# cold-deuu/Quadrotor_Manipulator_MPPI

Measured on AMD Instinct MI355X. Metric: MPPI rollouts/sec (K x H state-steps) + control-step p50 latency, K=4096 H=32, higher is better.
Workload: dtype f32

## Files before the change

quadrotor_manipulator_mppi_amd/csrc/mppi_finalize.hip:

```cpp
#include <algorithm>

#include "mppi_device.h"

using namespace mppi;

constexpr int kFinThreads = 512;
constexpr int kMaxRec = 4096;
#ifndef MPPI_FIN_KO
#define MPPI_FIN_KO 0
#endif
#ifndef MPPI_FIN_NOMARK
#define MPPI_FIN_NOMARK 0
#endif
#ifndef MPPI_FIN_XCDS
#define MPPI_FIN_XCDS 8
#endif
#ifndef MPPI_FIN_QUIET_LEAN
#define MPPI_FIN_QUIET_LEAN 1
#endif

#if defined(MPPI_STAMPS) && !defined(MPPI_TIMELINE)
#define FSTAMP(i)                                                                    \
    do {                                                                             \
        __builtin_amdgcn_sched_barrier(0);                                           \
        if (pk.stamps && threadIdx.x == 0)                                           \
            pk.stamps[(((size_t)v * A + a) * ts + sl) * kStamps + (i)] =               \
                __builtin_amdgcn_s_memtime();                                        \
        __builtin_amdgcn_sched_barrier(0);                                           \
    } while (0)
#define FSTAMPRT(i) do { } while (0)
#elif defined(MPPI_STAMPS)
#define FSTAMPRT(i)                                                                  \
    do {                                                                             \
        if (pk.stamps && threadIdx.x == 0) {                                         \
            pk.stamps[(((size_t)v * A + a) * ts + sl) * kStamps + (i)] =               \
                __builtin_amdgcn_s_memrealtime();                                    \
            if ((i) == 13)                                                           \
                pk.stamps[(((size_t)v * A + a) * ts + sl) * kStamps + 15] =            \
                    (unsigned long long)__builtin_amdgcn_s_getreg(0xF814);           \
        }                                                                            \
    } while (0)
#define FSTAMP(i) do { if ((i) == 1 || (i) == 7) FSTAMPRT(i); } while (0)
#else
#define FSTAMP(i) do { } while (0)
#define FSTAMPRT(i) do { } while (0)
#endif

enum { kRoleAny = 0, kRoleFinal = 1, kRoleQuiet = 2, kRolePack = 3, kRolePeer = 4 };
struct GeoRt { static constexpr bool kStatic = false; static constexpr int A = 0, H = 0, tsz = 0, hf = 0, ts = 0; };
template <int A_, int H_, int TSZ_, int HF_, int TS_>
struct GeoC { static constexpr bool kStatic = true; static constexpr int A = A_, H = H_, tsz = TSZ_, hf = HF_, ts = TS_; };

template <int CW, int WIN, int NT, int ROLE, typename GEO, int CPL = 1>
__device__ __forceinline__ void fin_body(const float* __restrict__ hdr_base, const float* __restrict__ dat_base,
                                         const FinTail* __restrict__ tail, const uint32_t nrec_H, const uint32_t geo,
                                         const int32_t hdr_rs, const int32_t d_rs, const int32_t d_as,
                                         const int32_t hdr_vs, const int32_t d_vs, const uint32_t seq_arg,
                                         const FinParams& pk) {
    constexpr bool kAny = ROLE == kRoleAny, kQuiet = ROLE == kRoleQuiet;
    constexpr bool kOut = kAny || ROLE == kRoleFinal || ROLE == kRolePeer;
    constexpr bool kUpd = kOut || kQuiet;
    constexpr bool kPeer = kAny || ROLE == kRolePeer;
    constexpr bool kEta2 = !(kQuiet && MPPI_FIN_QUIET_LEAN);
    constexpr int NWV = NT / 64;
    constexpr int ROWS = 64 / CW;
    constexpr int TR = NWV * ROWS;
    constexpr int kNPT = 16;
    static_assert(CPL == 1 || ((CPL == 2 || CPL == 4) && CW == 16 && NT / CPL >= 32), "lane maps: see above");
    constexpr int LPR = CW / CPL;
    constexpr int kLanes = NT / CPL < 64 ? NT / CPL : 64;
    __shared__ float wcol[NWV][CW];
    __shared__ float wrho[NWV], wnan[NWV], weta[NWV], weta2[NWV];
    __shared__ float wsg[96];
    const FinParams& p = pk;
    const int tid = threadIdx.x, lane = tid & 63, wv = tid >> 6;
    const int n = (int)(nrec_H & 0xFFFFu);
    const int H = GEO::kStatic ? GEO::H : (int)(nrec_H >> 16);
    const int tsz = GEO::kStatic ? GEO::tsz : (int)(geo & 0xFFu), hf = GEO::kStatic ? GEO::hf : (int)((geo >> 8) & 0xFFu);
    const int ts = GEO::kStatic ? GEO::ts : (int)((geo >> 16) & 0xFFu), A = GEO::kStatic ? GEO::A : (int)(geo >> 24);
    const int x8 = blockIdx.x & 7, j8 = blockIdx.x >> 3, na = (A + MPPI_FIN_XCDS - 1) / MPPI_FIN_XCDS;
    const int sl = (na == 1) ? j8 : (na == 2) ? (j8 >> 1) : j8 / na;
    const int a = x8 + MPPI_FIN_XCDS * (j8 - sl * na), v = blockIdx.y;
    if (x8 >= MPPI_FIN_XCDS || a >= A) return;
    if (MPPI_FIN_KO & 16) { if (tid == 0) p.u_prev[blockIdx.x] = 0.0f; return; }
    FSTAMPRT(13);
    FSTAMP(0);
// ... 94 lines not shown
            }
            if (wv == 0 && xpeers)
                xpl = ((const __attribute__((address_space(1))) unsigned long long*)xpeers)[lane < xn ? lane : 0];
        }
    };
    float rho_t = INFINITY, nanflag = 0.0f, eta = 0.0f, eta2 = 0.0f;
    float acc[CPL];
#pragma unroll
    for (int j = 0; j < CPL; ++j) acc[j] = 0.0f;
    const uint32_t hrs_b = (uint32_t)hdr_rs * 4u, drs_b = (uint32_t)d_rs * 4u;
    const __amdgpu_buffer_rsrc_t hrsrc =
        __builtin_amdgcn_make_buffer_rsrc(const_cast<float*>(hdr), 0, __builtin_amdgcn_readfirstlane((int)((uint32_t)n * hrs_b)),
                                          0x00020000);
    const __amdgpu_buffer_rsrc_t crsrc = __builtin_amdgcn_make_buffer_rsrc(
        const_cast<float*>(col), 0,
        __builtin_amdgcn_readfirstlane((int)((uint32_t)(n - 1) * drs_b + (uint32_t)(CPL == 1 ? W : nqd * CPL) * 4u)),
        0x00020000);
    typedef uint32_t u32x4 __attribute__((ext_vector_type(4)));
    typedef uint32_t u32x2 __attribute__((ext_vector_type(2)));
    for (int base = 0; base < n; base += TR * kNPT) {
        float4 hd[kNPT];
        float xv[kNPT][CPL];
        uint32_t okm = 0;
        const uint32_t r0 = (uint32_t)(base + gr);
        const uint32_t hoff = r0 * hrs_b, coff = r0 * drs_b + (uint32_t)(qv ? q : 0) * (uint32_t)(4 * CPL);
#pragma unroll
        for (int i = 0; i < kNPT; ++i) {
            okm |= (uint32_t)(r0 + (uint32_t)(i * TR) < (uint32_t)n) << i;
            const u32x4 h = __builtin_amdgcn_raw_buffer_load_b128(hrsrc, (int)(hoff + (uint32_t)(i * TR) * hrs_b), 0, kAuxDev);
            hd[i] = make_float4(__uint_as_float(h.x), __uint_as_float(h.y), __uint_as_float(h.z), __uint_as_float(h.w));
            const int bo = (int)(coff + (uint32_t)(i * TR) * drs_b);
            if constexpr (CPL == 4) {
                const u32x4 b = __builtin_amdgcn_raw_buffer_load_b128(crsrc, bo, 0, kAuxDev);
                xv[i][0] = __uint_as_float(b.x); xv[i][1] = __uint_as_float(b.y);
                xv[i][2] = __uint_as_float(b.z); xv[i][3] = __uint_as_float(b.w);
            } else if constexpr (CPL == 2) {
                const u32x2 b = __builtin_amdgcn_raw_buffer_load_b64(crsrc, bo, 0, kAuxDev);
                xv[i][0] = __uint_as_float(b.x); xv[i][1] = __uint_as_float(b.y);
            } else {
                xv[i][0] = __uint_as_float(__builtin_amdgcn_raw_buffer_load_b32(crsrc, bo, 0, kAuxDev));
            }
        }
        if (base == 0) {
            __builtin_amdgcn_sched_barrier(0);
            pin_tail();
        }
#pragma unroll
        for (int i = 0; i < kNPT; ++i)
            if (!((okm >> i) & 1u)) hd[i].x = INFINITY;
        FSTAMP(7);
        float m = INFINITY;
#pragma unroll
        for (int i = 0; i < kNPT; ++i) { m = fminf(m, hd[i].x); nanflag = fmaxf(nanflag, hd[i].w); }
        if constexpr (!kEta2) {
#pragma unroll
            for (int i = 0; i < kNPT; ++i) asm volatile("" :: "v"(hd[i].z));
        }
        float fr[kNPT];
#pragma unroll
        for (int i = 0; i < kNPT; ++i) fr[i] = 0.0f;
        if (m < INFINITY) {
            const float rn = fminf(rho_t, m);
            if (rho_t < INFINITY) {
                const float sc = __expf(coef * (rho_t - rn));
#pragma unroll
                for (int j = 0; j < CPL; ++j) acc[j] *= sc;
                eta *= sc;
                if constexpr (kEta2) eta2 *= sc * sc;
            }
            rho_t = rn;
#pragma unroll
            for (int i = 0; i < kNPT; ++i) {
                const float f = (hd[i].x < INFINITY) ? __expf(coef * (hd[i].x - rn)) : 0.0f;
                fr[i] = f;
                eta = fmaf(f, hd[i].y, eta);
                if constexpr (kEta2) eta2 = fmaf(f * f, hd[i].z, eta2);
            }
        }
#pragma unroll
        for (int i = 0; i < kNPT; ++i) {
#pragma unroll
            for (int j = 0; j < CPL; ++j) acc[j] = fmaf(fr[i], xv[i][j], acc[j]);
        }
        FSTAMP(8);
    }
    if constexpr (CPL == 1) {
        const float rw = fold_rows<CW>(rho_t, OpMin());
        const float sc = (rho_t < INFINITY) ? __expf(coef * (rho_t - rw)) : 0.0f;
        acc[0] = fold_rows<CW>(acc[0] * sc, OpAdd());
        const float e1 = fold_rows<CW>(eta * sc, OpAdd()), e2 = fold_rows<CW>(eta2 * (sc * sc), OpAdd());
        const float nf = fold_rows<CW>(nanflag, OpMax());
        if (lane < CW) wcol[wv][lane] = acc[0];
        if (lane == 0) { wrho[wv] = rw; wnan[wv] = nf; weta[wv] = e1; weta2[wv] = e2; }
    } else {
        auto fold_g = [](float x, auto op) {
            asm volatile("" : "+v"(x));
// ... 434 lines not shown
```

quadrotor_manipulator_mppi_amd/csrc/mppi_host_math.cpp:

```cpp
#include <algorithm>
#include <cmath>
#include <cstdarg>
#include <cstdio>
#include <cstring>
#include <string>
#include <vector>

#include "mppi_engine.h"

using namespace mppi;

namespace {
thread_local std::string g_err;

template <typename T>
void base_from_xyzquat_t(const double* b, float* T16) {
    const T qx = (T)b[3], qy = (T)b[4], qz = (T)b[5], qw = (T)b[6];
    volatile T a, c;
    std::memset(T16, 0, 16 * sizeof(float));
    a = (T)1 - (T)2 * (qy * qy); a = a - (T)2 * (qz * qz); T16[0] = (float)a;
    a = ((T)2 * qx) * qy; c = ((T)2 * qz) * qw; T16[1] = (float)(a - c);
    a = ((T)2 * qx) * qz; c = ((T)2 * qy) * qw; T16[2] = (float)(a + c);
    a = ((T)2 * qx) * qy; c = ((T)2 * qz) * qw; T16[4] = (float)(a + c);
    a = (T)1 - (T)2 * (qx * qx); a = a - (T)2 * (qz * qz); T16[5] = (float)a;
// ... 219 lines not shown
        if (!(c.quad_mass > 0.0f) || !(c.quad_inertia[0] > 0.0f) || !(c.quad_inertia[1] > 0.0f) ||
            !(c.quad_inertia[2] > 0.0f))
            return fail(MPPI_ERR_INVALID_ARG, "QUADROTOR needs a positive mass and inertia");
    }
    if (c.model == MPPI_MODEL_ARM || c.model == MPPI_MODEL_WHOLEBODY) {
        if (c.n_joints < 1 || c.n_joints > MPPI_MAX_JOINTS)
            return fail(MPPI_ERR_INVALID_ARG, "n_joints=%d", c.n_joints);
        const int nq = nq_of(c);
        for (int j = 0; j < c.n_joints; ++j) {
            const mppi_joint& jj = c.joints[j];
            if (jj.type < 0 || jj.type > 2) return fail(MPPI_ERR_INVALID_ARG, "joint %d: bad type", j);
            if (jj.type != MPPI_JOINT_FIXED && (jj.q_index < 0 || jj.q_index >= nq))
                return fail(MPPI_ERR_INVALID_ARG, "joint %d: q_index %d outside [0,%d)", j, jj.q_index, nq);
        }
    }
    const int half = c.savgol_window / 2;
    if (c.savgol_window % 2 != 1 || c.savgol_window > kMaxW)
        return fail(MPPI_ERR_INVALID_ARG, "Window size must be odd (and <= %d).", kMaxW);
    if (c.savgol_order >= c.savgol_window)
        return fail(MPPI_ERR_INVALID_ARG, "Polyorder must be less than window size.");
    if (c.n_horizon <= half)
        return fail(MPPI_ERR_INVALID_ARG, "Padding (%d) is too large for data length (%d).", half, c.n_horizon);
    if (!(c.lambda_ > 0.0) || !(c.dt > 0.0)) return fail(MPPI_ERR_INVALID_ARG, "lambda and dt must be > 0");
    if (c.shard_count < 1 || c.shard_rank < 0 || c.shard_rank >= c.shard_count)
        return fail(MPPI_ERR_INVALID_ARG, "shard %d/%d", c.shard_rank, c.shard_count);
    if ((int64_t)c.shard_count * (int64_t)c.n_samples > (int64_t)1 << 32)
        return fail(MPPI_ERR_INVALID_ARG, "shard_count %d x n_samples %d = %lld samples: the 32-bit sample counter of "
                    "the noise stream addresses at most 2^32", c.shard_count, c.n_samples,
                    (long long)c.shard_count * (long long)c.n_samples);
    if (c.vehicle_offset < 0 || c.vehicle_offset + c.n_vehicles > 32768)
        return fail(MPPI_ERR_INVALID_ARG, "vehicle_offset %d: the fleet-wide vehicle index must stay below 32768",
                    c.vehicle_offset);
    if (c.cost_terms & ~0x3F) return fail(MPPI_ERR_INVALID_ARG, "unknown cost_terms bits 0x%x", c.cost_terms);
    if ((c.cost_terms & 0x1F) && (c.model == MPPI_MODEL_DRONE || c.model == MPPI_MODEL_QUADROTOR))
        return fail(MPPI_ERR_INVALID_ARG, "cost_terms apply to the ARM / WHOLEBODY CostManager (not DRONE)");
    if (c.block_threads && (c.block_threads % 64 || c.block_threads > 512))
        return fail(MPPI_ERR_INVALID_ARG, "block_threads must be a multiple of 64 <= 512");
    return MPPI_OK;
}

}

using namespace mppi_host;

extern "C" {

// ... 122 lines not shown
```

quadrotor_manipulator_mppi_amd/csrc/mppi_rollout.h:

```cpp
#pragma once
#include "mppi_device.h"

#ifndef MPPI_KO
#define MPPI_KO 0
#endif
#ifndef MPPI_ROLL_OCC_NCH2
#define MPPI_ROLL_OCC_NCH2 4
#endif
#ifndef MPPI_ROLL_OCC_NCH2_XC
#define MPPI_ROLL_OCC_NCH2_XC 2
#endif
#ifndef MPPI_ROLL_OCC_XC
#define MPPI_ROLL_OCC_XC 4
#endif
#ifndef MPPI_ROLL_OCC
#define MPPI_ROLL_OCC 4
#endif
#ifndef MPPI_PRIO
#define MPPI_PRIO 1
#endif
#ifndef MPPI_S_PLAIN
#define MPPI_S_PLAIN 0
#endif
#ifndef MPPI_EPS_STASH
#define MPPI_EPS_STASH 1
#endif
#ifndef MPPI_COMB_EXIT
#define MPPI_COMB_EXIT 0
#endif
#ifndef MPPI_QUIET_LEAN
#define MPPI_QUIET_LEAN 1
#endif
#ifndef MPPI_FK_PRETRIG
#define MPPI_FK_PRETRIG 1
#endif

namespace {

__device__ __forceinline__ uint32_t xor3_sk(uint32_t a, uint32_t b, uint32_t k) {
    uint32_t r;
    asm("v_bitop3_b32 %0, %1, %2, %3 bitop3:0x96" : "=v"(r) : "v"(a), "v"(b), "s"(k));
    return r;
}

__device__ __forceinline__ void philox10(uint32_t& c0, uint32_t& c1, uint32_t& c2, uint32_t& c3,
                                         uint32_t k0, uint32_t k1) {
    k0 = __builtin_amdgcn_readfirstlane(k0);
    k1 = __builtin_amdgcn_readfirstlane(k1);
#pragma unroll
    for (int r = 0; r < 10; ++r) {
        if (r) {
            asm volatile("s_add_u32 %0, %0, 0x9e3779b9" : "+s"(k0) :: "scc");
            asm volatile("s_add_u32 %0, %0, 0xbb67ae85" : "+s"(k1) :: "scc");
        }
        const uint64_t p0 = (uint64_t)0xD2511F53u * c0;
        const uint64_t p1 = (uint64_t)0xCD9E8D57u * c2;
        const uint32_t n0 = xor3_sk((uint32_t)(p1 >> 32), c1, k0), n2 = xor3_sk((uint32_t)(p0 >> 32), c3, k1);
        c0 = n0; c1 = (uint32_t)p1; c2 = n2; c3 = (uint32_t)p0;
    }
// ... 520 lines not shown
#pragma unroll
        for (int j = 0; j < NU; ++j)
            ur[j] = __uint_as_float(__builtin_amdgcn_raw_buffer_load_b32(urs, (tid + j * nthr) * 4, 0, kAuxDev));
    };
    if (!ovl) load_u();
    if (MODEL != MPPI_MODEL_DRONE) {
        const int* js = (const int*)jtab;
#pragma unroll
        for (int j = 0; j < NJ; ++j) {
            const int i = tid + j * nthr;
            jr[j] = (i < kJW) ? js[i] : 0;
        }
    }
    constexpr int kVCW = (int)(sizeof(VehicleConst) / 4);
    const int vcr = (tid < kVCW) ? (VONE ? ((const int*)&pk.vc0)[tid] : ((const int*)(pk.vc + v))[tid]) : 0;
    float tgt[TRK ? NCH : 1][12];
    if constexpr (TRK) {
#pragma unroll
        for (int c = 0; c < NCH; ++c) {
            const int t = t0 + 64 * c, tc = (t < H_arg) ? t : H_arg - 1;
            load_target_row<MODEL == MPPI_MODEL_DRONE>(ttab + ((size_t)v * H_arg + tc) * 12, tgt[c]);
        }
    }
    uint32_t kwarm = 0u;
    {
        const uint32_t* kp = (const uint32_t*)&pk;
#pragma unroll
        for (int o = 0; o < (int)(offsetof(DevParams, sigma) / 4); o += 16) kwarm ^= kp[o];
    }
    STAMPW(9);
    float z0[NCH][NA];
    SECTION("prologue_philox");
    if (noise_mode != MPPI_NOISE_INJECTED) {
        const uint32_t kg = k_off + (uint32_t)((blockIdx.x * nw + wid) * R + sub);
#pragma unroll
        for (int c = 0; c < NCH; ++c)
            draw_normals<NA>(z0[c], kg, (uint32_t)(t0 + 64 * c), vkey, step_ctr, seed_lo, seed_hi);
    }
    if (ovl) {
        if (wid == 0) {
            const uint32_t* fl = pk.ovl + (size_t)v * pk.ovl_n;
            const int nfl = pk.ovl_n;
            for (;;) {
                bool ok = true;
                for (int i = lane; i < nfl; i += 64) ok &= (int32_t)(ld_dev(fl + i) - step_ctr) >= 0;
                if (__builtin_amdgcn_ballot_w64(!ok) == 0ull) break;
                __builtin_amdgcn_s_sleep(1);
            }
        }
        lds_barrier();
        load_u();
    }
    SECTION("prologue_staging");
    STAMP(10);
    asm volatile("" :: "s"(kwarm));
#pragma unroll
    for (int j = 0; j < NU; ++j) {
        const int i = tid + j * nthr;
        if (i < HA) u_lds[i] = ur[j];
    }
    if constexpr (!B512)
        for (int i = tid + 4 * nthr; i < HA; i += nthr) u_lds[i] = usrc[i];
    if (MODEL != MPPI_MODEL_DRONE) {
#pragma unroll
        for (int j = 0; j < NJ; ++j) {
            const int i = tid + j * nthr;
            if (i < kJW) ((int*)jnt)[i] = jr[j];
        }
        if constexpr (!B512)
            for (int i = tid + 2 * nthr; i < kJW; i += nthr) ((int*)jnt)[i] = ((const int*)jtab)[i];
    }
    if (tid < kVCW) {
        ((int*)&vcv)[tid] = vcr;
        if (kHand && VONE && blockIdx.x == 0)
            __hip_atomic_store((int*)pk.vc + tid, tid == kVcStepWord ? (int)step_ctr : vcr, __ATOMIC_RELAXED,
                               __HIP_MEMORY_SCOPE_AGENT);
    }
    if constexpr (!B512) {
        for (int i = tid + nthr; i < kVCW; i += nthr) {
            const int x = VONE ? ((const int*)&pk.vc0)[i] : ((const int*)(pk.vc + v))[i];
            ((int*)&vcv)[i] = x;
            if (kHand && VONE && blockIdx.x == 0)
                __hip_atomic_store((int*)pk.vc + i, i == kVcStepWord ? (int)step_ctr : x, __ATOMIC_RELAXED,
                                   __HIP_MEMORY_SCOPE_AGENT);
        }
    }
    STAMPW(8);
    if (!(MPPI_KO & 256)) lds_barrier();
    const VehicleConst& vc = vcv;
    const float* sdiag = pk.sdiag;
    const int H = H_arg, K = pk.K;
    constexpr int kWs = wave_slot_floats<NA, NCH, LSEG>();
    float* const xw = smem + ((HA + 3) & ~3) + wid * kWs;
    float* const s_stage = smem + ((HA + 3) & ~3) + 8 * kWs;
    STAMP(1);

    const int hp = kTraj ? pk.hp : 0;
    const uint32_t plane_b = (uint32_t)K * (uint32_t)hp * 4u;
    const __amdgpu_buffer_rsrc_t trs = traj_rsrc(kTraj ? pk.traj + (size_t)v * pk.C * K * hp : nullptr, plane_b,
                                                 kTraj ? pk.C : 0);

    float acc[NCH][NA];
#pragma unroll
    for (int c = 0; c < NCH; ++c)
#pragma unroll
        for (int a = 0; a < NA; ++a) acc[c][a] = 0.0f;
    float rho_w = INFINITY, eta_w = 0.0f, eta2_w = 0.0f;
    bool nan_w = false;

    auto group = [&](const int it) __attribute__((always_inline)) {
        asm volatile("" ::: "memory");
        SECTION("noise");
        const int g = blockIdx.x + it * p.nb;
        const int k = (g * nw + wid) * R + sub;
        const bool kval = k < K;
        const int kc = kval ? k : K - 1;
        const uint32_t kg = k_off + (uint32_t)k;

        float eps[NCH][NA], act[NCH][NA];
#pragma unroll
        for (int c = 0; c < NCH; ++c) {
            const int t = t0 + 64 * c;
            const bool val = kval && t < H;
            const int tc = (t < H) ? t : H - 1;
            if (noise_mode == MPPI_NOISE_INJECTED) {
                const float* src = p.noise_in + (((size_t)v * K + kc) * H + tc) * NA;
#pragma unroll
                for (int a = 0; a < NA; ++a) eps[c][a] = src[a];
            } else {
                float z[NA];
                if (it == 0) {
#pragma unroll
                    for (int a = 0; a < NA; ++a) z[a] = z0[c][a];
                } else {
                    draw_normals<NA>(z, kg, (uint32_t)t, vkey, step_ctr, seed_lo, seed_hi);
                }
                if (!XC || p.sigma_diag) {
#pragma unroll
                    for (int a = 0; a < NA; ++a) eps[c][a] = z[a] * sdiag[a];
                } else {
#pragma unroll
                    for (int b = 0; b < NA; ++b) {
                        float e = 0.0f;
#pragma unroll
                        for (int a = 0; a < NA; ++a) e += z[a] * p.sigma[a * NA + b];
                        eps[c][b] = e;
                    }
                }
            }
            float ur[NA];
#pragma unroll
            for (int a = 0; a < NA; ++a) ur[a] = u_lds[tc * NA + a];
#pragma unroll
            for (int a = 0; a < NA; ++a) {
                eps[c][a] = val ? eps[c][a] : 0.0f;
                act[c][a] = val ? ur[a] + eps[c][a] : 0.0f;
            }
            if (!QUIET && p.store_noise && val) {
                float* dst = p.noise_out + (((size_t)v * K + k) * H + t) * NA;
#pragma unroll
                for (int a = 0; a < NA; ++a) st_dev(dst + a, eps[c][a]);
            }
        }
        float ecov = 0.0f, eact = 0.0f, gts[NCH];
#pragma unroll
        for (int c = 0; c < NCH; ++c) gts[c] = 0.0f;
        if (XC && (TRK ? (p.cost_terms & ~MPPI_COST_TARGET_TRACK) : p.cost_terms)) {
#pragma unroll
            for (int c = 0; c < NCH; ++c) {
                const int t = t0 + 64 * c;
                const bool val = kval && t < H;
                const int tc = (t < H) ? t : H - 1;
                gts[c] = val ? p.gamma_t[tc] : 0.0f;
                if (p.cost_terms & MPPI_COST_COVAR) {
                    float qd = 0.0f;
#pragma unroll
                    for (int a = 0; a < NA; ++a) {
                        float y = 0.0f;
                        if (p.sigma_diag) {
                            y = p.sinv[a * NA + a] * act[c][a];
                        } else {
#pragma unroll
                            for (int b = 0; b < NA; ++b) y = fmaf(p.sinv[a * NA + b], act[c][b], y);
                        }
                        qd = fmaf(u_lds[tc * NA + a], y, qd);
                    }
                    ecov += val ? qd : 0.0f;
                }
                if (p.cost_terms & MPPI_COST_ACTION) {
                    float s2 = 0.0f;
#pragma unroll
                    for (int a = 0; a < NA; ++a) s2 = fmaf(act[c][a], act[c][a], s2);
                    eact += val ? (p.w_act * s2) * gts[c] : 0.0f;
                }
            }
        }
        if (it == 0) STAMP(2);
        SECTION("integrator");

        float posf[NCH][NA];
        double posd[NCH][F64 ? NA : 1];
        if constexpr (NCH == 1 && !(MPPI_KO & 1)) {
            float inc[NA];
            integrate_lds<LSEG, NA>(act[0], xw, lane, p.dt, 0.5f * p.dt2, vc.vel0f, inc);
#pragma unroll
            for (int a = 0; a < NA; ++a) {
                if (!F64) {
                    posf[0][a] = inc[a] + vc.pos0f[a];
                } else {
                    posd[0][a] = (double)inc[a] + vc.pos0[a];
                    posf[0][a] = (float)posd[0][a];
                }
            }
        } else {
#pragma clang fp contract(off)
            float carry1[NA], carry2[NA], lastv[NA];
#pragma unroll
            for (int a = 0; a < NA; ++a) { carry1[a] = 0.0f; carry2[a] = 0.0f; lastv[a] = 0.0f; }
#pragma unroll
            for (int c = 0; c < NCH; ++c) {
                float c1[NA], c2[NA];
#pragma unroll
                for (int a = 0; a < NA; ++a) c1[a] = act[c][a] * p.dt;
                seg_scan_f32_multi<LSEG, NA>(c1);
#pragma unroll
                for (int a = 0; a < NA; ++a) {
                    if (NCH > 1) {
                        c1[a] += carry1[a];
                        carry1[a] = read_lane_f32(c1[a], 63);
                    }
                    const float h2 = act[c][a] * (0.5f * p.dt2);
                    const float velf = c1[a] + vc.vel0f[a];
                    float prev = dpp_f32<0x138, 0xF>(velf);
                    if (t0 == 0) prev = (c == 0) ? vc.vel0f[a] : lastv[a];
                    if (NCH > 1) lastv[a] = read_lane_f32(velf, 63);
                    c2[a] = prev * p.dt + h2;
                }
                seg_scan_f32_multi<LSEG, NA>(c2);
#pragma unroll
                for (int a = 0; a < NA; ++a) {
                    if (NCH > 1) {
                        c2[a] += carry2[a];
                        carry2[a] = read_lane_f32(c2[a], 63);
                    }
                    if (!F64) {
                        posf[c][a] = c2[a] + vc.pos0f[a];
                    } else {
                        posd[c][a] = (double)c2[a] + vc.pos0[a];
                        posf[c][a] = (float)posd[c][a];
                    }
                }
            }
        }
        if (it == 0) STAMP(3);
        SECTION("fk_chain");
        if (ONEG && MPPI_PRIO) set_wave_prio(2);

        constexpr bool kStash = MPPI_EPS_STASH && NA >= 7 && (XC || NCH > 1);
        constexpr int kESP = (NCH == 1) ? IntegGeom<LSEG, NA>::P : NA;
        if constexpr (kStash) {
#pragma unroll
            for (int c = 0; c < NCH; ++c)
#pragma unroll
                for (int a = 0; a < NA; ++a) xw[(c * 64 + lane) * kESP + a] = eps[c][a];
            asm volatile("" ::: "memory");
        }

        float xs[NCH];
        float ecen = 0.0f, ejt = 0.0f, elim = 0.0f;
#pragma unroll
        for (int c = 0; c < NCH; ++c) {
            const int t = t0 + 64 * c;
            const bool val = kval && t < H;
            const bool term = (t == H - 1);
            float x;
            const uint32_t toff = ((uint32_t)k * (uint32_t)hp + (uint32_t)t) * 4u;
            const bool stv = kTraj && p.store_traj && kval && t < hp;
            if (MODEL == MPPI_MODEL_DRONE) {
                const float dx = posf[c][0] - (TRK ? tgt[c][0] : vc.tpos[0]), dy = posf[c][1] - (TRK ? tgt[c][1] : vc.tpos[1]),
                            dz = posf[c][2] - (TRK ? tgt[c][2] : vc.tpos[2]);
                x = dx * dx + dy * dy + dz * dz;
                if (stv) {
#pragma unroll
                    for (int a = 0; a < 3; ++a) traj_store(trs, toff, (uint32_t)a * plane_b, posf[c][a]);
                }
            } else {
                auto qang = [&](int cc_, int j) {
                    if constexpr (F64) return posd[cc_][QOFF + j]; else return posf[cc_][QOFF + j];
                };
                if (stv) {
#pragma unroll
                    for (int a = 0; a < NA; ++a) traj_store(trs, toff, (uint32_t)a * plane_b, posf[c][a]);
                }
                Mat34 T;
#pragma unroll
                for (int i = 0; i < 12; ++i) T.m[i] = vc.base[i];
                if (MODEL == MPPI_MODEL_WHOLEBODY) {
                    T.m[3] += posf[c][0]; T.m[7] += posf[c][1]; T.m[11] += posf[c][2];
                }
                if (MPPI_KO & 4) {
                    T.m[3] += posf[c][QOFF]; T.m[7] += posf[c][QOFF + 1];
                } else if (NQ == 7 && (!XC || p.chain_fast == 2)) {
                    if constexpr (MPPI_FK_PRETRIG && !XC && NCH == 1 && F64 && LSEG == 32 && MODEL == MPPI_MODEL_ARM) {
                        float sj[7], cj[7];
#pragma unroll
                        for (int j = 0; j < 7; ++j) sincos_joint(qang(c, j), sj[j], cj[j]);
                        __builtin_amdgcn_sched_barrier(0);
                        kin_joint_sc<0>(T, jnt[p.j0 + 0].O, sj[0], cj[0]);
                        kin_joint_sc<1>(T, jnt[p.j0 + 1].O, sj[1], cj[1]);
                        kin_joint_sc<2>(T, jnt[p.j0 + 2].O, sj[2], cj[2]);
                        kin_joint_sc<3>(T, jnt[p.j0 + 3].O, sj[3], cj[3]);
                        kin_joint_sc<4>(T, jnt[p.j0 + 4].O, sj[4], cj[4]);
                        kin_joint_sc<5>(T, jnt[p.j0 + 5].O, sj[5], cj[5]);
                        kin_joint_sc<6>(T, jnt[p.j0 + 6].O, sj[6], cj[6]);
                    } else {
                        kin_joint<0>(T, jnt[p.j0 + 0].O, qang(c, 0));
                        kin_joint<1>(T, jnt[p.j0 + 1].O, qang(c, 1));
                        kin_joint<2>(T, jnt[p.j0 + 2].O, qang(c, 2));
                        kin_joint<3>(T, jnt[p.j0 + 3].O, qang(c, 3));
                        kin_joint<4>(T, jnt[p.j0 + 4].O, qang(c, 4));
                        kin_joint<5>(T, jnt[p.j0 + 5].O, qang(c, 5));
                        kin_joint<6>(T, jnt[p.j0 + 6].O, qang(c, 6));
                    }
                } else if (!XC) {
                } else if (p.chain_fast) {
#pragma unroll
                    for (int j = 0; j < NQ; ++j) {
                        const JointDev& J = jnt[p.j0 + j];
                        mul_affine(T, J.O);
                        float s, cc;
                        sincos_joint(qang(c, j), s, cc);
                        const float omc = 1.0f - cc, r22 = cc + omc;
#pragma unroll
                        for (int i = 0; i < 3; ++i) {
                            const float a0 = T.m[4 * i], a1 = T.m[4 * i + 1];
                            T.m[4 * i] = a0 * cc + a1 * s;
                            T.m[4 * i + 1] = a1 * cc - a0 * s;
                            T.m[4 * i + 2] = T.m[4 * i + 2] * r22;
                        }
                    }
                } else {
                    for (int jn = p.j0; jn < p.nj; ++jn) {
                        const JointDev& J = jnt[jn];
                        mul_affine(T, J.O);
                        if (J.type == MPPI_JOINT_FIXED) continue;
                        double qd = 0.0;
                        float qf = 0.0f;
#pragma unroll
                        for (int a = 0; a < NQ; ++a)
                            if (a == J.q_index) {
                                qd = F64 ? posd[c][QOFF + a] : 0.0;
                                qf = posf[c][QOFF + a];
                            }
                        if (J.type == MPPI_JOINT_REVOLUTE) {
                            float s, cc;
                            if constexpr (F64) sincos_joint(qd, s, cc); else sincos_joint(qf, s, cc);
                            mul_revolute(T, J, cc, s);
                        } else {
                            mul_prismatic(T, J, qf);
                        }
                    }
                }
                const float wsp = uniform_f32(p.w_sp), wso = uniform_f32(p.w_so), wtp = uniform_f32(p.w_tp),
                            wto = uniform_f32(p.w_to);
                SECTION("pose_cost");
                if constexpr (TRK) x = pose_cost_row(T, tgt[c], term ? wtp : wsp, term ? wto : wso);
                else x = (MPPI_KO & 8) ? T.m[3] + T.m[7] + T.m[11] + T.m[0] : pose_cost(T, vc, term ? wtp : wsp, term ? wto : wso);
                SECTION("traj_ee_stores");
                if (stv) {
#pragma unroll
                    for (int i = 0; i < 12; ++i) traj_store(trs, toff, (uint32_t)(NA + i) * plane_b, T.m[i]);
                }
            }
            xs[c] = val ? x : 0.0f;
            if (XC && (p.cost_terms & (MPPI_COST_CENTER | MPPI_COST_JOINT_TRACK | MPPI_COST_JOINT_LIMIT))) {
                const int tc = (t < H) ? t : H - 1;
                const float* jt = p.jtraj ? p.jtraj + ((size_t)v * H + tc) * NQ : nullptr;
                float sc = 0.0f, sj = 0.0f;
                bool out = false;
#pragma unroll
                for (int j = 0; j < NQ; ++j) {
                    const float qj = posf[c][QOFF + j];
                    const float dc = qj - vc.qc[j];
                    sc = fmaf(dc, dc, sc);
                    const float dj = qj - (jt ? jt[j] : 0.0f);
                    sj = fmaf(dj, dj, sj);
                    const double qd = F64 ? posd[c][QOFF + j] : (double)qj;
// ... 4 lines not shown
                    if (p.cost_terms & MPPI_COST_JOINT_TRACK) ejt += (p.w_jt * sj) * gts[c];
                    if ((p.cost_terms & MPPI_COST_JOINT_LIMIT) && out) elim += p.lim_pen * gts[c];
                }
            }
        }
        if (it == 0) STAMP(4);
        SECTION("cost_sum_softmin");
        if (ONEG && MPPI_PRIO) set_wave_prio(1);

        float st = 0.0f;
#pragma unroll
        for (int c = 0; c < NCH; ++c) st += (t0 + 64 * c < H - 1) ? xs[c] : 0.0f;
        st = seg_scan_f32<LSEG>(st);
        float xt = 0.0f;
#pragma unroll
        for (int c = 0; c < NCH; ++c)
            if (c == (H - 1) / 64) xt = xs[c];
        float S_seg[R];
#pragma unroll
        for (int s = 0; s < R; ++s) {
            const int ks = (g * nw + wid) * R + s;
            const float stage = read_lane_f32(st, s * LSEG + LSEG - 1);
            const float term = read_lane_f32(xt, s * LSEG + ((H - 1) & 63));
            float S = (MODEL == MPPI_MODEL_DRONE) ? (p.w_sp * stage) + (p.w_tp * term) : stage + term;
            S_seg[s] = (ks < K) ? S : INFINITY;
        }
        if (XC) {
            float tsum[5] = {ecov, ecen, ejt, eact, elim};
            const int bits[5] = {MPPI_COST_COVAR, MPPI_COST_CENTER, MPPI_COST_JOINT_TRACK, MPPI_COST_ACTION,
                                 MPPI_COST_JOINT_LIMIT};
#pragma unroll
            for (int i = 0; i < 5; ++i) {
                if (!(p.cost_terms & bits[i])) continue;
                const float ts = seg_scan_f32<LSEG>(tsum[i]);
#pragma unroll
                for (int s = 0; s < R; ++s) {
                    float add = read_lane_f32(ts, s * LSEG + LSEG - 1);
                    if (i == 0) add = p.w_cov * add;
                    S_seg[s] += add;
                }
            }
        }
        float S_mine = S_seg[0];
#pragma unroll
        for (int s = 1; s < R; ++s) S_mine = (sub == s) ? S_seg[s] : S_mine;
        if (!kCosts) { }
        else if (MPPI_S_PLAIN) { if (kval && t0 == 0) p.S[(size_t)v * K + k] = S_mine; }
        else if (kval && t0 == 0) s_stage[it * cost_run_stride(nw * R) + wid * R + sub] = S_mine;

        float m = INFINITY;
#pragma unroll
        for (int s = 0; s < R; ++s) {
            const bool bad = S_seg[s] != S_seg[s];
            nan_w |= bad;
            if (!bad) m = fminf(m, S_seg[s]);
        }
        if (m < INFINITY) {
            const float rn = fminf(rho_w, m);
            const float f = (rho_w == INFINITY) ? 0.0f : __expf(p.coef * (rho_w - rn));
            float es = 0.0f, e2 = 0.0f;
#pragma unroll
            for (int s = 0; s < R; ++s) {
                const float e = (S_seg[s] < INFINITY) ? __expf(p.coef * (S_seg[s] - rn)) : 0.0f;
                es += e;
                if constexpr (kEta2) e2 += e * e;
            }
            eta_w = eta_w * f + es;
            if constexpr (kEta2) eta2_w = eta2_w * f * f + e2;
            const float e_mine = (kval && !(S_mine != S_mine)) ? __expf(p.coef * (S_mine - rn)) : 0.0f;
            if constexpr (kStash) {
                asm volatile("" ::: "memory");
#pragma unroll
                for (int c = 0; c < NCH; ++c)
#pragma unroll
                    for (int a = 0; a < NA; ++a) eps[c][a] = xw[(c * 64 + lane) * kESP + a];
            }
#pragma unroll
            for (int c = 0; c < NCH; ++c)
#pragma unroll
                for (int a = 0; a < NA; ++a) acc[c][a] = acc[c][a] * f + e_mine * eps[c][a];
            rho_w = rn;
        }
    };
    if (ONEG) {
        if (MPPI_PRIO) set_wave_prio(3);
        group(0);
        if (MPPI_PRIO) set_wave_prio(0);
    } else if (iters == 1) {
        group(0);
    } else {
        for (int it = 0; it < iters; ++it) {
            if (MPPI_PRIO) set_wave_prio(iters - 1 - it);
            group(it);
        }
        if (MPPI_PRIO) set_wave_prio(0);
    }
    STAMP(5);
    SECTION("block_combine_record");

    float* wsh = smem + ((HA + 3) & ~3);
    const int wstride = kWs;
    float* mine = wsh + wid * wstride;
    if (lane == 0) {
        mine[0] = rho_w; mine[1] = eta_w; mine[2] = eta2_w; mine[3] = nan_w ? 1.0f : 0.0f;
    }
    if constexpr (!B512)
        for (int i = nw * wstride + tid; i < 8 * wstride; i += nthr)
            wsh[i] = ((i - nw * wstride) % wstride == 0) ? INFINITY : 0.0f;
#pragma unroll
    for (int c = 0; c < NCH; ++c)
#pragma unroll
        for (int a = 0; a < NA; ++a) mine[4 + (c * 64 + lane) * NA + a] = acc[c][a];
    STAMPW(11);
    lds_barrier();
    STAMP(6);
    if (kCosts && !MPPI_S_PLAIN && wid == nw - 1) {
        const int nS = nw * R, q = (nS + 3) >> 2;
        float* const Sv = uniform_ptr(p.S + (size_t)v * K);
        for (int i = lane; i < iters * q; i += 64) {
            const int it = i / q, k0 = (blockIdx.x + it * p.nb) * nS;
            st_dev_run(Sv, (uint32_t)k0, s_stage + it * cost_run_stride(nS), min(nS, K - k0), i - it * q);
        }
    }
    if (MPPI_COMB_EXIT && wid != 0 && wid * 64 >= HA) {
        drain_stores();
        return;
    }
    float rws[8], rho_b = INFINITY;
#pragma unroll
    for (int w = 0; w < 8; ++w) {
        rws[w] = wsh[w * wstride];
        rho_b = fminf(rho_b, rws[w]);
    }
    float fw[8];
    {
        float mine = INFINITY;
#pragma unroll
        for (int w = 0; w < 8; ++w) mine = ((lane & 7) == w) ? rws[w] : mine;
        const float f = (mine < INFINITY) ? __expf(p.coef * (mine - rho_b)) : 0.0f;
#pragma unroll
        for (int w = 0; w < 8; ++w) fw[w] = read_lane_f32(f, w);
    }
    STAMP(12);
    if (tid == 0) {
        float eta = 0.0f, eta2 = 0.0f, nanf = 0.0f;
#pragma unroll
        for (int w = 0; w < 8; ++w) {
            eta += fw[w] * wsh[w * wstride + 1];
            if constexpr (kEta2) eta2 += fw[w] * fw[w] * wsh[w * wstride + 2];
            nanf = fmaxf(nanf, wsh[w * wstride + 3]);
        }
        wt_store4(uniform_ptr(p.hdr), ((uint32_t)v * (uint32_t)p.nb + blockIdx.x) * 16u, make_float4(rho_b, eta, eta2, nanf));
    }
    const float rH = __builtin_amdgcn_rcpf((float)H);
    float* const rdata_v = uniform_ptr(p.rdata + (size_t)v * NA * p.nb * H);
    const uint32_t rbase = blockIdx.x * (uint32_t)H;
    const uint32_t rstride = (uint32_t)p.nb * (uint32_t)H;
    for (int i = tid; i < ((MPPI_KO & 64) ? 0 : HA); i += nthr) {
        const int a = (int)(((float)i + 0.5f) * rH), t = i - a * H;
        const int c = t >> 6, tl = t & 63;
        float s = 0.0f;
#pragma unroll
        for (int w = 0; w < 8; ++w) {
            float sw = wsh[w * wstride + 4 + (c * 64 + tl) * NA + a];
#pragma unroll
            for (int sg = 1; sg < R; ++sg) sw += wsh[w * wstride + 4 + (c * 64 + sg * LSEG + tl) * NA + a];
            s += fw[w] * sw;
        }
        wt_store(rdata_v, (rbase + (uint32_t)a * rstride + (uint32_t)t) * 4u, s);
    }
    STAMP(7);
    STAMPRT(14);
    drain_stores();
}

template <int MODEL, int NA, int NCH, int LSEG, bool F64, bool VONE, bool XC, bool ONEG>
__global__ void __launch_bounds__(512, (roll_occ<NCH, F64, XC, ONEG>())) k_rollout(const uint32_t seed_lo, const uint32_t seed_hi,
                                                 const uint32_t step_arg, const uint32_t k_off,
                                                 const int32_t noise_arg, const int32_t H_arg,
                                                 const int32_t geo_arg,
                                                 const float* __restrict__ u_prev,
                                                 const JointDev* __restrict__ jtab, const DevParams pk) {
    rollout_body<MODEL, NA, NCH, LSEG, F64, VONE, XC, ONEG, false>(seed_lo, seed_hi, step_arg, k_off, noise_arg, H_arg,
                                                                   geo_arg, u_prev, jtab, pk);
}
template <int MODEL, int NA, int NCH, int LSEG, bool F64, bool VONE, bool XC>
__global__ void __launch_bounds__(512, (roll_occ<NCH, F64, XC, true>())) k_rollout_s(const uint32_t seed_lo, const uint32_t seed_hi,
                                                 const uint32_t step_arg, const uint32_t k_off,
                                                 const int32_t noise_arg, const int32_t H_arg,
                                                 const int32_t geo_arg,
                                                 const float* __restrict__ u_prev,
                                                 const JointDev* __restrict__ jtab, const DevParams pk) {
    rollout_body<MODEL, NA, NCH, LSEG, F64, VONE, XC, true, true>(seed_lo, seed_hi, step_arg, k_off, noise_arg, H_arg,
                                                                  geo_arg, u_prev, jtab, pk);
}

// ... 129 lines not shown
```

Measured before the change: 18.20 billion.

## Pin hot kernel params in SGPRs and skip tail masking on full chunks

In the rollout kernel, frequently used kernel-argument fields (K, nb, dt, coef, weights, pointers, noise scales) are loaded once into scalar registers and pinned with asm constraints. This replaces repeated kernarg loads and the old warm-up read. The combine epilogue's header and output base offsets are now computed before the barrier. In finalize, the per-row validity mask is skipped for full chunks, and the INFINITY guard before expf is dropped. A host-side check rejects lambda values whose -1/lambda underflows in f32, so the unguarded exp still yields zero for infinite costs. The cost is higher SGPR pressure.

```diff
diff --git a/quadrotor_manipulator_mppi_amd/csrc/mppi_finalize.hip b/quadrotor_manipulator_mppi_amd/csrc/mppi_finalize.hip
--- a/quadrotor_manipulator_mppi_amd/csrc/mppi_finalize.hip
+++ b/quadrotor_manipulator_mppi_amd/csrc/mppi_finalize.hip
@@ -17,6 +17,12 @@
 #endif
 #ifndef MPPI_FIN_QUIET_LEAN
 #define MPPI_FIN_QUIET_LEAN 1
+#endif
+#ifndef MPPI_FIN_FULL_CHUNK
+#define MPPI_FIN_FULL_CHUNK 1
+#endif
+#ifndef MPPI_FIN_EXP_BARE
+#define MPPI_FIN_EXP_BARE 1
 #endif
 
 #if defined(MPPI_STAMPS) && !defined(MPPI_TIMELINE)
@@ -62,6 +68,7 @@
     constexpr bool kUpd = kOut || kQuiet;
     constexpr bool kPeer = kAny || ROLE == kRolePeer;
     constexpr bool kEta2 = !(kQuiet && MPPI_FIN_QUIET_LEAN);
+    constexpr bool kFull = MPPI_FIN_FULL_CHUNK && !kPeer;
     constexpr int NWV = NT / 64;
     constexpr int ROWS = 64 / CW;
     constexpr int TR = NWV * ROWS;
@@ -202,11 +209,12 @@
         float4 hd[kNPT];
         float xv[kNPT][CPL];
         uint32_t okm = 0;
+        const bool ragged = !kFull || base + TR * kNPT > n;
         const uint32_t r0 = (uint32_t)(base + gr);
         const uint32_t hoff = r0 * hrs_b, coff = r0 * drs_b + (uint32_t)(qv ? q : 0) * (uint32_t)(4 * CPL);
 #pragma unroll
         for (int i = 0; i < kNPT; ++i) {
-            okm |= (uint32_t)(r0 + (uint32_t)(i * TR) < (uint32_t)n) << i;
+            if constexpr (!kFull) okm |= (uint32_t)(r0 + (uint32_t)(i * TR) < (uint32_t)n) << i;
             const u32x4 h = __builtin_amdgcn_raw_buffer_load_b128(hrsrc, (int)(hoff + (uint32_t)(i * TR) * hrs_b), 0, kAuxDev);
             hd[i] = make_float4(__uint_as_float(h.x), __uint_as_float(h.y), __uint_as_float(h.z), __uint_as_float(h.w));
             const int bo = (int)(coff + (uint32_t)(i * TR) * drs_b);
@@ -225,9 +233,15 @@
             __builtin_amdgcn_sched_barrier(0);
             pin_tail();
         }
-#pragma unroll
-        for (int i = 0; i < kNPT; ++i)
-            if (!((okm >> i) & 1u)) hd[i].x = INFINITY;
+        if (ragged) {
+            if constexpr (kFull) {
+#pragma unroll
+                for (int i = 0; i < kNPT; ++i) okm |= (uint32_t)(r0 + (uint32_t)(i * TR) < (uint32_t)n) << i;
+            }
+#pragma unroll
+            for (int i = 0; i < kNPT; ++i)
+                if (!((okm >> i) & 1u)) hd[i].x = INFINITY;
+        }
         FSTAMP(7);
         float m = INFINITY;
 #pragma unroll
@@ -251,7 +265,8 @@
             rho_t = rn;
 #pragma unroll
             for (int i = 0; i < kNPT; ++i) {
-                const float f = (hd[i].x < INFINITY) ? __expf(coef * (hd[i].x - rn)) : 0.0f;
+                const float f = MPPI_FIN_EXP_BARE ? __expf(coef * (hd[i].x - rn))
+                                                  : (hd[i].x < INFINITY) ? __expf(coef * (hd[i].x - rn)) : 0.0f;
                 fr[i] = f;
                 eta = fmaf(f, hd[i].y, eta);
                 if constexpr (kEta2) eta2 = fmaf(f * f, hd[i].z, eta2);
diff --git a/quadrotor_manipulator_mppi_amd/csrc/mppi_host_math.cpp b/quadrotor_manipulator_mppi_amd/csrc/mppi_host_math.cpp
--- a/quadrotor_manipulator_mppi_amd/csrc/mppi_host_math.cpp
+++ b/quadrotor_manipulator_mppi_amd/csrc/mppi_host_math.cpp
@@ -265,6 +265,8 @@
     if (c.n_horizon <= half)
         return fail(MPPI_ERR_INVALID_ARG, "Padding (%d) is too large for data length (%d).", half, c.n_horizon);
     if (!(c.lambda_ > 0.0) || !(c.dt > 0.0)) return fail(MPPI_ERR_INVALID_ARG, "lambda and dt must be > 0");
+    if (!((float)(-1.0 / c.lambda_) < 0.0f))
+        return fail(MPPI_ERR_INVALID_ARG, "lambda %g: -1/lambda underflows single precision", c.lambda_);
     if (c.shard_count < 1 || c.shard_rank < 0 || c.shard_rank >= c.shard_count)
         return fail(MPPI_ERR_INVALID_ARG, "shard %d/%d", c.shard_rank, c.shard_count);
     if ((int64_t)c.shard_count * (int64_t)c.n_samples > (int64_t)1 << 32)
diff --git a/quadrotor_manipulator_mppi_amd/csrc/mppi_rollout.h b/quadrotor_manipulator_mppi_amd/csrc/mppi_rollout.h
--- a/quadrotor_manipulator_mppi_amd/csrc/mppi_rollout.h
+++ b/quadrotor_manipulator_mppi_amd/csrc/mppi_rollout.h
@@ -34,7 +34,12 @@
 #ifndef MPPI_FK_PRETRIG
 #define MPPI_FK_PRETRIG 1
 #endif
-
+#ifndef MPPI_ROLL_PIN
+#define MPPI_ROLL_PIN 1
+#endif
+#ifndef MPPI_COMB_PRE
+#define MPPI_COMB_PRE 1
+#endif
 namespace {
 
 __device__ __forceinline__ uint32_t xor3_sk(uint32_t a, uint32_t b, uint32_t k) {
@@ -601,11 +606,30 @@
             load_target_row<MODEL == MPPI_MODEL_DRONE>(ttab + ((size_t)v * H_arg + tc) * 12, tgt[c]);
         }
     }
+    constexpr bool kRoom = ONEG && !XC && (B512 || F64);
+    constexpr bool kPin = MPPI_ROLL_PIN && kRoom;
     uint32_t kwarm = 0u;
-    {
+    if constexpr (!kPin) {
         const uint32_t* kp = (const uint32_t*)&pk;
 #pragma unroll
         for (int o = 0; o < (int)(offsetof(DevParams, sigma) / 4); o += 16) kwarm ^= kp[o];
+    }
+#define HOT(m) (kPin ? s_##m : pk.m)
+    int32_t s_K = 0, s_nb = 0, s_j0 = 0, s_hp = 0, s_C = 0, s_store_traj = 0, s_store_noise = 0;
+    float s_dt = 0.0f, s_dt2 = 0.0f, s_coef = 0.0f, s_w_sp = 0.0f, s_w_so = 0.0f, s_w_tp = 0.0f, s_w_to = 0.0f, s_sdiag[NA];
+    float *s_hdr = nullptr, *s_rdata = nullptr, *s_traj = nullptr, *s_S = nullptr, *s_noise_out = nullptr;
+    const float* s_noise_in = nullptr;
+#pragma unroll
+    for (int a = 0; a < NA; ++a) s_sdiag[a] = kPin ? pk.sdiag[a] : 0.0f;
+    if constexpr (kPin) {
+        s_K = pk.K; s_nb = pk.nb; s_j0 = pk.j0;
+        s_dt = pk.dt; s_dt2 = pk.dt2; s_coef = pk.coef;
+        s_w_sp = pk.w_sp; s_w_so = pk.w_so; s_w_tp = pk.w_tp; s_w_to = pk.w_to;
+        s_hdr = pk.hdr; s_rdata = pk.rdata; s_noise_in = pk.noise_in;
+        if constexpr (!QUIET) {
+            s_hp = pk.hp; s_C = pk.C; s_store_traj = pk.store_traj; s_store_noise = pk.store_noise;
+            s_traj = pk.traj; s_S = pk.S; s_noise_out = pk.noise_out;
+        }
     }
     STAMPW(9);
     float z0[NCH][NA];
@@ -632,7 +656,24 @@
     }
     SECTION("prologue_staging");
     STAMP(10);
-    asm volatile("" :: "s"(kwarm));
+    if constexpr (kPin) {
+        asm volatile("" : "+s"(s_K), "+s"(s_nb), "+s"(s_j0), "+s"(s_dt), "+s"(s_dt2), "+s"(s_coef), "+s"(s_w_sp), "+s"(s_w_so),
+                          "+s"(s_w_tp), "+s"(s_w_to), "+s"(s_hdr), "+s"(s_rdata), "+s"(s_noise_in));
+        if constexpr (!QUIET)
+            asm volatile("" : "+s"(s_hp), "+s"(s_C), "+s"(s_store_traj), "+s"(s_store_noise), "+s"(s_traj), "+s"(s_S),
+                              "+s"(s_noise_out));
+        if constexpr (NA == 3) asm volatile("" : "+s"(s_sdiag[0]), "+s"(s_sdiag[1]), "+s"(s_sdiag[2]));
+        else if constexpr (NA == 7)
+            asm volatile("" : "+s"(s_sdiag[0]), "+s"(s_sdiag[1]), "+s"(s_sdiag[2]), "+s"(s_sdiag[3]), "+s"(s_sdiag[4]),
+                              "+s"(s_sdiag[5]), "+s"(s_sdiag[6]));
+        else {
+            static_assert(NA == 10, "pin the noise scales of a new action width here");
+            asm volatile("" : "+s"(s_sdiag[0]), "+s"(s_sdiag[1]), "+s"(s_sdiag[2]), "+s"(s_sdiag[3]), "+s"(s_sdiag[4]),
+                              "+s"(s_sdiag[5]), "+s"(s_sdiag[6]), "+s"(s_sdiag[7]), "+s"(s_sdiag[8]), "+s"(s_sdiag[9]));
+        }
+    } else {
+        asm volatile("" :: "s"(kwarm));
+    }
 #pragma unroll
     for (int j = 0; j < NU; ++j) {
         const int i = tid + j * nthr;
@@ -667,17 +708,16 @@
     STAMPW(8);
     if (!(MPPI_KO & 256)) lds_barrier();
     const VehicleConst& vc = vcv;
-    const float* sdiag = pk.sdiag;
-    const int H = H_arg, K = pk.K;
+    const int H = H_arg, K = HOT(K);
     constexpr int kWs = wave_slot_floats<NA, NCH, LSEG>();
     float* const xw = smem + ((HA + 3) & ~3) + wid * kWs;
     float* const s_stage = smem + ((HA + 3) & ~3) + 8 * kWs;
     STAMP(1);
 
-    const int hp = kTraj ? pk.hp : 0;
+    const int hp = kTraj ? HOT(hp) : 0;
     const uint32_t plane_b = (uint32_t)K * (uint32_t)hp * 4u;
-    const __amdgpu_buffer_rsrc_t trs = traj_rsrc(kTraj ? pk.traj + (size_t)v * pk.C * K * hp : nullptr, plane_b,
-                                                 kTraj ? pk.C : 0);
+    const __amdgpu_buffer_rsrc_t trs = traj_rsrc(kTraj ? HOT(traj) + (size_t)v * HOT(C) * K * hp : nullptr, plane_b,
+                                                 kTraj ? HOT(C) : 0);
 
     float acc[NCH][NA];
 #pragma unroll
@@ -690,7 +730,7 @@
     auto group = [&](const int it) __attribute__((always_inline)) {
         asm volatile("" ::: "memory");
         SECTION("noise");
-        const int g = blockIdx.x + it * p.nb;
+        const int g = blockIdx.x + it * HOT(nb);
         const int k = (g * nw + wid) * R + sub;
         const bool kval = k < K;
         const int kc = kval ? k : K - 1;
@@ -703,7 +743,7 @@
             const bool val = kval && t < H;
             const int tc = (t < H) ? t : H - 1;
             if (noise_mode == MPPI_NOISE_INJECTED) {
-                const float* src = p.noise_in + (((size_t)v * K + kc) * H + tc) * NA;
+                const float* src = HOT(noise_in) + (((size_t)v * K + kc) * H + tc) * NA;
 #pragma unroll
                 for (int a = 0; a < NA; ++a) eps[c][a] = src[a];
             } else {
@@ -716,7 +756,7 @@
                 }
                 if (!XC || p.sigma_diag) {
 #pragma unroll
-                    for (int a = 0; a < NA; ++a) eps[c][a] = z[a] * sdiag[a];
+                    for (int a = 0; a < NA; ++a) eps[c][a] = z[a] * (kPin ? s_sdiag[a] : pk.sdiag[a]);
                 } else {
 #pragma unroll
                     for (int b = 0; b < NA; ++b) {
@@ -735,8 +775,8 @@
                 eps[c][a] = val ? eps[c][a] : 0.0f;
                 act[c][a] = val ? ur[a] + eps[c][a] : 0.0f;
             }
-            if (!QUIET && p.store_noise && val) {
-                float* dst = p.noise_out + (((size_t)v * K + k) * H + t) * NA;
+            if (!QUIET && HOT(store_noise) && val) {
+                float* dst = HOT(noise_out) + (((size_t)v * K + k) * H + t) * NA;
 #pragma unroll
                 for (int a = 0; a < NA; ++a) st_dev(dst + a, eps[c][a]);
             }
@@ -781,7 +821,7 @@
         double posd[NCH][F64 ? NA : 1];
         if constexpr (NCH == 1 && !(MPPI_KO & 1)) {
             float inc[NA];
-            integrate_lds<LSEG, NA>(act[0], xw, lane, p.dt, 0.5f * p.dt2, vc.vel0f, inc);
+            integrate_lds<LSEG, NA>(act[0], xw, lane, HOT(dt), 0.5f * HOT(dt2), vc.vel0f, inc);
 #pragma unroll
             for (int a = 0; a < NA; ++a) {
                 if (!F64) {
@@ -800,7 +840,7 @@
             for (int c = 0; c < NCH; ++c) {
                 float c1[NA], c2[NA];
 #pragma unroll
-                for (int a = 0; a < NA; ++a) c1[a] = act[c][a] * p.dt;
+                for (int a = 0; a < NA; ++a) c1[a] = act[c][a] * HOT(dt);
                 seg_scan_f32_multi<LSEG, NA>(c1);
 #pragma unroll
                 for (int a = 0; a < NA; ++a) {
@@ -808,12 +848,12 @@
                         c1[a] += carry1[a];
                         carry1[a] = read_lane_f32(c1[a], 63);
                     }
-                    const float h2 = act[c][a] * (0.5f * p.dt2);
+                    const float h2 = act[c][a] * (0.5f * HOT(dt2));
                     const float velf = c1[a] + vc.vel0f[a];
                     float prev = dpp_f32<0x138, 0xF>(velf);
                     if (t0 == 0) prev = (c == 0) ? vc.vel0f[a] : lastv[a];
                     if (NCH > 1) lastv[a] = read_lane_f32(velf, 63);
-                    c2[a] = prev * p.dt + h2;
+                    c2[a] = prev * HOT(dt) + h2;
                 }
                 seg_scan_f32_multi<LSEG, NA>(c2);
 #pragma unroll
@@ -854,7 +894,7 @@
             const bool term = (t == H - 1);
             float x;
             const uint32_t toff = ((uint32_t)k * (uint32_t)hp + (uint32_t)t) * 4u;
-            const bool stv = kTraj && p.store_traj && kval && t < hp;
+            const bool stv = kTraj && HOT(store_traj) && kval && t < hp;
             if (MODEL == MPPI_MODEL_DRONE) {
                 const float dx = posf[c][0] - (TRK ? tgt[c][0] : vc.tpos[0]), dy = posf[c][1] - (TRK ? tgt[c][1] : vc.tpos[1]),
                             dz = posf[c][2] - (TRK ? tgt[c][2] : vc.tpos[2]);
@@ -885,27 +925,27 @@
 #pragma unroll
                         for (int j = 0; j < 7; ++j) sincos_joint(qang(c, j), sj[j], cj[j]);
                         __builtin_amdgcn_sched_barrier(0);
-                        kin_joint_sc<0>(T, jnt[p.j0 + 0].O, sj[0], cj[0]);
-                        kin_joint_sc<1>(T, jnt[p.j0 + 1].O, sj[1], cj[1]);
-                        kin_joint_sc<2>(T, jnt[p.j0 + 2].O, sj[2], cj[2]);
-                        kin_joint_sc<3>(T, jnt[p.j0 + 3].O, sj[3], cj[3]);
-                        kin_joint_sc<4>(T, jnt[p.j0 + 4].O, sj[4], cj[4]);
-                        kin_joint_sc<5>(T, jnt[p.j0 + 5].O, sj[5], cj[5]);
-                        kin_joint_sc<6>(T, jnt[p.j0 + 6].O, sj[6], cj[6]);
+                        kin_joint_sc<0>(T, jnt[HOT(j0) + 0].O, sj[0], cj[0]);
+                        kin_joint_sc<1>(T, jnt[HOT(j0) + 1].O, sj[1], cj[1]);
+                        kin_joint_sc<2>(T, jnt[HOT(j0) + 2].O, sj[2], cj[2]);
+                        kin_joint_sc<3>(T, jnt[HOT(j0) + 3].O, sj[3], cj[3]);
+                        kin_joint_sc<4>(T, jnt[HOT(j0) + 4].O, sj[4], cj[4]);
+                        kin_joint_sc<5>(T, jnt[HOT(j0) + 5].O, sj[5], cj[5]);
+                        kin_joint_sc<6>(T, jnt[HOT(j0) + 6].O, sj[6], cj[6]);
                     } else {
-                        kin_joint<0>(T, jnt[p.j0 + 0].O, qang(c, 0));
-                        kin_joint<1>(T, jnt[p.j0 + 1].O, qang(c, 1));
-                        kin_joint<2>(T, jnt[p.j0 + 2].O, qang(c, 2));
-                        kin_joint<3>(T, jnt[p.j0 + 3].O, qang(c, 3));
-                        kin_joint<4>(T, jnt[p.j0 + 4].O, qang(c, 4));
-                        kin_joint<5>(T, jnt[p.j0 + 5].O, qang(c, 5));
-                        kin_joint<6>(T, jnt[p.j0 + 6].O, qang(c, 6));
+                        kin_joint<0>(T, jnt[HOT(j0) + 0].O, qang(c, 0));
+                        kin_joint<1>(T, jnt[HOT(j0) + 1].O, qang(c, 1));
+                        kin_joint<2>(T, jnt[HOT(j0) + 2].O, qang(c, 2));
+                        kin_joint<3>(T, jnt[HOT(j0) + 3].O, qang(c, 3));
+                        kin_joint<4>(T, jnt[HOT(j0) + 4].O, qang(c, 4));
+                        kin_joint<5>(T, jnt[HOT(j0) + 5].O, qang(c, 5));
+                        kin_joint<6>(T, jnt[HOT(j0) + 6].O, qang(c, 6));
                     }
                 } else if (!XC) {
                 } else if (p.chain_fast) {
 #pragma unroll
                     for (int j = 0; j < NQ; ++j) {
-                        const JointDev& J = jnt[p.j0 + j];
+                        const JointDev& J = jnt[HOT(j0) + j];
                         mul_affine(T, J.O);
                         float s, cc;
                         sincos_joint(qang(c, j), s, cc);
@@ -919,7 +959,7 @@
                         }
                     }
                 } else {
-                    for (int jn = p.j0; jn < p.nj; ++jn) {
+                    for (int jn = HOT(j0); jn < p.nj; ++jn) {
                         const JointDev& J = jnt[jn];
                         mul_affine(T, J.O);
                         if (J.type == MPPI_JOINT_FIXED) continue;
@@ -940,8 +980,8 @@
                         }
                     }
                 }
-                const float wsp = uniform_f32(p.w_sp), wso = uniform_f32(p.w_so), wtp = uniform_f32(p.w_tp),
-                            wto = uniform_f32(p.w_to);
+                const float wsp = uniform_f32(HOT(w_sp)), wso = uniform_f32(HOT(w_so)), wtp = uniform_f32(HOT(w_tp)),
+                            wto = uniform_f32(HOT(w_to));
                 SECTION("pose_cost");
                 if constexpr (TRK) x = pose_cost_row(T, tgt[c], term ? wtp : wsp, term ? wto : wso);
                 else x = (MPPI_KO & 8) ? T.m[3] + T.m[7] + T.m[11] + T.m[0] : pose_cost(T, vc, term ? wtp : wsp, term ? wto : wso);
@@ -992,7 +1032,7 @@
             const int ks = (g * nw + wid) * R + s;
             const float stage = read_lane_f32(st, s * LSEG + LSEG - 1);
             const float term = read_lane_f32(xt, s * LSEG + ((H - 1) & 63));
-            float S = (MODEL == MPPI_MODEL_DRONE) ? (p.w_sp * stage) + (p.w_tp * term) : stage + term;
+            float S = (MODEL == MPPI_MODEL_DRONE) ? (HOT(w_sp) * stage) + (HOT(w_tp) * term) : stage + term;
             S_seg[s] = (ks < K) ? S : INFINITY;
         }
         if (XC) {
@@ -1015,7 +1055,7 @@
 #pragma unroll
         for (int s = 1; s < R; ++s) S_mine = (sub == s) ? S_seg[s] : S_mine;
         if (!kCosts) { }
-        else if (MPPI_S_PLAIN) { if (kval && t0 == 0) p.S[(size_t)v * K + k] = S_mine; }
+        else if (MPPI_S_PLAIN) { if (kval && t0 == 0) HOT(S)[(size_t)v * K + k] = S_mine; }
         else if (kval && t0 == 0) s_stage[it * cost_run_stride(nw * R) + wid * R + sub] = S_mine;
 
         float m = INFINITY;
@@ -1027,17 +1067,17 @@
         }
         if (m < INFINITY) {
             const float rn = fminf(rho_w, m);
-            const float f = (rho_w == INFINITY) ? 0.0f : __expf(p.coef * (rho_w - rn));
+            const float f = (rho_w == INFINITY) ? 0.0f : __expf(HOT(coef) * (rho_w - rn));
             float es = 0.0f, e2 = 0.0f;
 #pragma unroll
             for (int s = 0; s < R; ++s) {
-                const float e = (S_seg[s] < INFINITY) ? __expf(p.coef * (S_seg[s] - rn)) : 0.0f;
+                const float e = (S_seg[s] < INFINITY) ? __expf(HOT(coef) * (S_seg[s] - rn)) : 0.0f;
                 es += e;
                 if constexpr (kEta2) e2 += e * e;
             }
             eta_w = eta_w * f + es;
             if constexpr (kEta2) eta2_w = eta2_w * f * f + e2;
-            const float e_mine = (kval && !(S_mine != S_mine)) ? __expf(p.coef * (S_mine - rn)) : 0.0f;
+            const float e_mine = (kval && !(S_mine != S_mine)) ? __expf(HOT(coef) * (S_mine - rn)) : 0.0f;
             if constexpr (kStash) {
                 asm volatile("" ::: "memory");
 #pragma unroll
@@ -1081,14 +1121,35 @@
     for (int c = 0; c < NCH; ++c)
 #pragma unroll
         for (int a = 0; a < NA; ++a) mine[4 + (c * 64 + lane) * NA + a] = acc[c][a];
+    constexpr bool kPre = MPPI_COMB_PRE && kRoom;
+    const uint32_t vz = (kPre && VONE) ? 0u : (uint32_t)v;
+    uint32_t hoff, rbase, rstride;
+    float *hdr_u, *rdata_v;
+    auto header_base = [&]() __attribute__((always_inline)) {
+        hoff = (vz * (uint32_t)HOT(nb) + blockIdx.x) * 16u;
+        hdr_u = uniform_ptr(HOT(hdr));
+    };
+    auto body_base = [&]() __attribute__((always_inline)) {
+        rdata_v = uniform_ptr(HOT(rdata) + (size_t)vz * NA * HOT(nb) * H);
+        rbase = blockIdx.x * (uint32_t)H;
+        rstride = (uint32_t)HOT(nb) * (uint32_t)H;
+    };
+    if constexpr (kPre) {
+        header_base();
+        body_base();
+        hoff = __builtin_amdgcn_readfirstlane(hoff);
+        rbase = __builtin_amdgcn_readfirstlane(rbase);
+        rstride = __builtin_amdgcn_readfirstlane(rstride);
+        asm volatile("" : "+s"(hoff), "+s"(hdr_u), "+s"(rdata_v), "+s"(rbase), "+s"(rstride));
+    }
     STAMPW(11);
     lds_barrier();
     STAMP(6);
     if (kCosts && !MPPI_S_PLAIN && wid == nw - 1) {
         const int nS = nw * R, q = (nS + 3) >> 2;
-        float* const Sv = uniform_ptr(p.S + (size_t)v * K);
+        float* const Sv = uniform_ptr(HOT(S) + (size_t)v * K);
         for (int i = lane; i < iters * q; i += 64) {
-            const int it = i / q, k0 = (blockIdx.x + it * p.nb) * nS;
+            const int it = i / q, k0 = (blockIdx.x + it * HOT(nb)) * nS;
             st_dev_run(Sv, (uint32_t)k0, s_stage + it * cost_run_stride(nS), min(nS, K - k0), i - it * q);
         }
     }
@@ -1107,7 +1168,7 @@
         float mine = INFINITY;
 #pragma unroll
         for (int w = 0; w < 8; ++w) mine = ((lane & 7) == w) ? rws[w] : mine;
-        const float f = (mine < INFINITY) ? __expf(p.coef * (mine - rho_b)) : 0.0f;
+        const float f = (mine < INFINITY) ? __expf(HOT(coef) * (mine - rho_b)) : 0.0f;
 #pragma unroll
         for (int w = 0; w < 8; ++w) fw[w] = read_lane_f32(f, w);
     }
@@ -1120,12 +1181,11 @@
             if constexpr (kEta2) eta2 += fw[w] * fw[w] * wsh[w * wstride + 2];
             nanf = fmaxf(nanf, wsh[w * wstride + 3]);
         }
-        wt_store4(uniform_ptr(p.hdr), ((uint32_t)v * (uint32_t)p.nb + blockIdx.x) * 16u, make_float4(rho_b, eta, eta2, nanf));
+        if constexpr (!kPre) header_base();
+        wt_store4(hdr_u, hoff, make_float4(rho_b, eta, eta2, nanf));
     }
     const float rH = __builtin_amdgcn_rcpf((float)H);
-    float* const rdata_v = uniform_ptr(p.rdata + (size_t)v * NA * p.nb * H);
-    const uint32_t rbase = blockIdx.x * (uint32_t)H;
-    const uint32_t rstride = (uint32_t)p.nb * (uint32_t)H;
+    if constexpr (!kPre) body_base();
     for (int i = tid; i < ((MPPI_KO & 64) ? 0 : HA); i += nthr) {
         const int a = (int)(((float)i + 0.5f) * rH), t = i - a * H;
         const int c = t >> 6, tl = t & 63;
@@ -1142,6 +1202,7 @@
     STAMP(7);
     STAMPRT(14);
     drain_stores();
+#undef HOT
 }
 
 template <int MODEL, int NA, int NCH, int LSEG, bool F64, bool VONE, bool XC, bool ONEG>
```

After: 19.02 billion, median of 6. 4.5% higher.
